# gdalsanto/flamo

Measured on AMD Instinct MI355X. Metric: freq-bin*channel products/sec (fwd+bwd), nfft=96000 8x8ch, higher is better.
Workload: dtype f32; 1 GPU; BASELINE configs[1]: Shell(FFT -> Series(Matrix 8x8, GEQ 8x8) -> iFFT), nfft=96000, batch 32 per GPU, fwd+bwd of (y**2).mean(), parameter grads; nfft=96000, channels=8, batch_per_gpu=32, parallelism=dp1 (batch), input_grad=False

## Files before the change

flamo_amd/_lib.py:

```python
from __future__ import annotations

import ctypes as C
import os
import subprocess
import threading

_HERE = os.path.dirname(os.path.abspath(__file__))
LIB_PATH = os.environ.get("FLAMO_HIP_LIB") or os.path.join(_HERE, "libflamo_hip.so")
CSRC = os.path.join(_HERE, "csrc")

_lock = threading.Lock()
_lib = None

_vp, _i, _l, _d, _sz = C.c_void_p, C.c_int, C.c_long, C.c_double, C.c_size_t

_SIGNATURES = {
    "fl_version": (_i, []),
    "fl_last_error": (C.c_char_p, []),
    "fl_twiddle_fill_f32": (_i, [_vp, _i, _vp]),
    "fl_twiddle_fill_f64": (_i, [_vp, _i, _vp]),
    "fl_fft_plan": (_i, [_i, _i, C.POINTER(_i), C.POINTER(_i)]),
    "fl_fft_scratch_elems": (_sz, [_i, _i, _i]),
    "fl_debug_set_fft_max_single": (_i, [_i]),
    "fl_debug_set_fft_fast": (_i, [_i]),
# ... 7 lines not shown
    "fl_spec_plan": (_i, [_i, C.POINTER(_i), C.POINTER(_i)]),
    "fl_spec_supports": (_i, [_i, _i, _i]),
    "fl_spec_supports_f64": (_i, [_i, _i, _i]),
    "fl_spec_aux_elems": (_sz, [_i]),
    "fl_spec_aux_fill_f32": (_i, [_vp, _i, _vp]),
    "fl_spec_aux_fill_f64": (_i, [_vp, _i, _vp]),
    "fl_debug_set_spec": (_i, [_i, _i]),
    "fl_debug_set_spec_times": (_i, [_vp]),
    "fl_spec_cols_fwd_f32": (_i, [_vp, _i, _i, _i, _vp, _vp, _i, _d, _vp]),
    "fl_spec_cols_fwd_f64": (_i, [_vp, _i, _i, _i, _vp, _vp, _i, _d, _vp]),
    "fl_spec_gradh_loop_supports_f32": (_i, [_i, _i, _i]),
    "fl_spec_gradh_loop_supports_f64": (_i, [_i, _i, _i]),
    "fl_spec_gradh_loop_f32": (_i, [_vp, _vp, _l, _l, _vp, _l, _l, _vp, _i, _i, _i, _i, _d, _i, _d, _vp, _vp]),
    "fl_spec_gradh_loop_f64": (_i, [_vp, _vp, _l, _l, _vp, _l, _l, _vp, _i, _i, _i, _i, _d, _i, _d, _vp, _vp]),
    "fl_spec_mid_f32": (_i, [_vp, _vp, _vp, _l, _l, _vp, _l, _l, _i, _vp, _i, _i, _i, _i, _d, _i, _i, _vp]),
    "fl_spec_mid_f64": (_i, [_vp, _vp, _vp, _l, _l, _vp, _l, _l, _i, _vp, _i, _i, _i, _i, _d, _i, _i, _vp]),
    "fl_spec_walk_supports": (_i, [_i, _i, _i]),
    "fl_spec_walk_spectrum_elems": (_sz, [_i, _i, _i]),
    "fl_spec_walk_workgroups": (_i, [_i, _i]),
    "fl_spec_walk_partition": (_i, [_i, _i, _i, C.POINTER(_i)]),
    "fl_spec_mid_walk_f32": (_i, [_vp, _vp, _vp, _vp, _l, _l, _i, _vp, _i, _i, _i, _i, _d, _i, _i, _vp, _vp]),
    "fl_spec_gradh_slices": (_i, [_i, _i]),
    "fl_spec_gradh_walk_f32": (_i, [_vp, _vp, _vp, _l, _l, _l, _i, _vp, _i, _i, _i, _i, _d, _i, _vp]),
    "fl_sum_parts_c64": (_i, [_vp, _l, _i, _vp, _l, _vp]),
    "fl_debug_set_walk": (_i, [_i, _i, _i, _vp]),
    "fl_debug_set_walk_stamps": (_i, [_vp]),
    "fl_wall_clock_khz": (_i, []),
    "fl_spec_cols_inv_f32": (_i, [_vp, _vp, _i, _i, _i, _i, _vp, _i, _d, _d, _vp]),
    "fl_spec_cols_inv_sumsq_f32": (_i, [_vp, _vp, _i, _i, _i, _i, _vp, _i, _d, _d, _vp, _vp]),
    "fl_spec_cols_inv_sumsq_f64": (_i, [_vp, _vp, _i, _i, _i, _i, _vp, _i, _d, _d, _vp, _vp]),
    "fl_spec_cols_blocks_f32": (_i, [_i, _i, _i]),
    "fl_spec_cols_blocks_f64": (_i, [_i, _i, _i]),
    "fl_spec_cols_inv_inplace_ok_f32": (_i, [_i, _i]),
    "fl_spec_cols_inv_inplace_ok_f64": (_i, [_i, _i]),
    "fl_spec_cols_inv_grad_supported_f32": (_i, [_i, _i]),
    "fl_spec_cols_inv_grad_supported_f64": (_i, [_i, _i]),
    "fl_spec_cols_inv_sumsq_grad_f32": (_i, [_vp, _vp, _vp, _i, _i, _vp, _i, _d, _vp, _vp]),
    "fl_spec_cols_inv_sumsq_grad_f64": (_i, [_vp, _vp, _vp, _i, _i, _vp, _i, _d, _vp, _vp]),
    "fl_spec_cols_inv_scaled_f32": (_i, [_vp, _vp, _i, _i, _i, _i, _vp, _i, _d, _vp, _d, _vp]),
    "fl_spec_cols_inv_scaled_f64": (_i, [_vp, _vp, _i, _i, _i, _i, _vp, _i, _d, _vp, _d, _vp]),
    "fl_spec_gradh_walk_scaled_f32": (_i, [_vp, _vp, _vp, _l, _l, _l, _i, _vp, _i, _i, _i, _i, _d, _i, _vp, _vp]),
    "fl_mean_square_final_f32": (_i, [_vp, _i, _d, _vp, _vp]),
    "fl_mean_square_final_f64": (_i, [_vp, _i, _d, _vp, _vp]),
    "fl_pack_toggle": (_i, [_vp, _i, _vp, _vp, _vp, _vp]),
    "fl_spec_cols_inv_f64": (_i, [_vp, _vp, _i, _i, _i, _i, _vp, _i, _d, _d, _vp]),
    "fl_permute_bins_c64": (_i, [_vp, _l, _vp, _l, _i, _i, _i, _vp]),
# ... 177 lines not shown
```

flamo_amd/csrc/specwalk.hip:

```cpp
#include "spectral_common.h"

namespace fl {
using namespace sp32;

struct WalkArgs {
    const cf* S;
    cf* S2;
    const cf* H;
    long hs_m, hs_n;
    int conj_h;
    const cf* W;
    int n, L, L1, L2, Bn;
    float spec_scale;
    int spec_interior2;
    int pre_half;
    const int* bounds;
    cf* Xp;
    long long* dbg_times;
    unsigned pol;
    long long* stamps;
};

__device__ __forceinline__ int opaque(int v) {
    asm volatile("" : "+v"(v));
// ... 392 lines not shown
        o[1] = clock64();
#pragma unroll
        for (int i = 0; i < 4; ++i) o[2 + i] = t_ph[i];
    }
    if (DBG && a.dbg_times && (tid == 0 || tid == 256))
        a.dbg_times[(size_t)blockIdx.x * 8 + 6 + grp] = grp == 0 && a.spec_interior2 == 7
            ? (q_ph[0] >> 4) | ((q_ph[1] >> 4) << 21) | ((q_ph[2] >> 4) << 42)
            : (w_ph[0] >> 4) | ((w_ph[1] >> 4) << 21) | ((w_ph[2] >> 4) << 42);
#undef FL_STAMP
}

struct GradhArgs {
    const cf* Sg;
    const cf* Xp;
    cf* dH;
    long ds_s, ds_m, ds_n;
    const cf* W;
    int n, L, L1, L2, Bn, NS;
    float scale_g;
    const float* out_scale;
    int interior2_g;
    long long* dbg_times;
    unsigned pol;
};

template <int A, int B, int NI, int NO, int NSC, int OCC, int DEPTH, bool DBG = false>
__global__ void __launch_bounds__(512, OCC) spec_gradh_walk(GradhArgs a) {
    extern __shared__ __attribute__((aligned(16))) char smem[];
    constexpr int LEN = A * B, LENP = walk_pitch(LEN);
    constexpr int NOL = NO / NSC;
    constexpr int UB = 2 * NOL * LENP;
    constexpr int NI1 = 2 * B * NOL, NI2 = 2 * NOL * A;
    constexpr int NW1 = (NI1 + 63) / 64;
    constexpr int SBG = NW1 * A * 64;
    constexpr int SBX = 8 * NI * 64;
    static_assert(LEN <= 256, "one bin pair per thread pair");
    static_assert(NO % NSC == 0 && NOL % 2 == 0 && NI % 2 == 0 && A % 2 == 0, "16-byte DMA granules");
    static_assert(NI1 <= 256 && NI2 <= 256, "an FFT stage of one unit fits one group");
    static_assert(DEPTH == 1 || DEPTH == 2, "one or two items in flight");
    constexpr int GA = A / 2, XA = NI / 2;
    constexpr int P2_OFF = 256 - ((NI2 + 63) / 64) * 64;
    cf* XF = reinterpret_cast<cf*>(smem);
    cf* Yb = XF + 2 * UB;
    cf* stage_g = Yb + UB;
    cf* stage_x = stage_g + DEPTH * SBG;
    constexpr int TWP = tw_pitch(A), TWL = (B * TWP + 1) & ~1;
    cf* tw = stage_x + DEPTH * SBX;
    cf* ws = tw + TWL;
    const int tid = threadIdx.x;
    const int wave = __builtin_amdgcn_readfirstlane(tid >> 6), lane = tid & 63;
    const int grp = wave >> 2;
    const int P = a.L1 / 2 + 1;
    const int xcd = blockIdx.x & 7, q_ = blockIdx.x >> 3;
    const int r = (q_ / (a.NS * NSC)) * 8 + xcd, sl = (q_ / NSC) % a.NS, mo = (q_ % NSC) * NOL;
    if (r >= P) return;
    const int rm = (a.L1 - r) % a.L1;
    const bool selfm = rm == r;
    const int b_lo = (int)((long)a.Bn * sl / a.NS), n_it = (int)((long)a.Bn * (sl + 1) / a.NS) - b_lo;
    const size_t bstride_g = (size_t)a.L1 * a.L2 * NO;
    const unsigned sg_lds = lds_addr_of(stage_g), sx_lds = lds_addr_of(stage_x);

    auto fetch_g = [&](int i, int cw) {
        const int b = b_lo + ((a.pol & POL_GRADH_FORWARD) ? i : n_it - 1 - i);
        const unsigned sg_buf = sg_lds + (unsigned)((i % DEPTH) * SBG * 8);
        const int hi = lane >> 5;
        int item0 = 64 * cw + 2 * (lane & 31);
        if (item0 >= NI1 || (item0 >= B * NOL && selfm)) item0 = 0;
        const int m0 = item0 % NOL, tb = (item0 / NOL) % B, slot = item0 / (NOL * B);
        const cf* src = a.Sg + (size_t)b * bstride_g + (size_t)(slot ? rm : r) * (a.L2 * NO) + ((hi * B + tb) * NO + mo + m0);
        if (a.pol & POL_GRADH_SG_NT) {
#pragma unroll
            for (int q = 0; q < A / 2; ++q) dma16p<true>(src + q * (2 * B * NO), sg_buf + (unsigned)(((cw * A + 2 * q) * 64) * 8));
        } else {
#pragma unroll
            for (int q = 0; q < A / 2; ++q) dma16p<false>(src + q * (2 * B * NO), sg_buf + (unsigned)(((cw * A + 2 * q) * 64) * 8));
        }
    };
    auto fetch_x = [&](int i, int cw) {
        const int b = b_lo + ((a.pol & POL_GRADH_FORWARD) ? i : n_it - 1 - i);
        const unsigned sx_buf = sx_lds + (unsigned)((i % DEPTH) * SBX * 8);
#if FL_XP_PAIRS
        int pp = 64 * (cw & 3) + lane;
        if (pp > LEN - 1) pp = LEN - 1;
        const cf* src = a.Xp + (((size_t)r * a.Bn + b) * 2 + (cw >> 2)) * (NI * LEN) + 2 * pp;
#else
        int pp = 64 * (cw & 3) + 2 * (lane & 31);
        if (pp > LEN - 2) pp = LEN - 2;
        const cf* src = a.Xp + (((size_t)r * a.Bn + b) * 2 + (cw >> 2)) * (NI * LEN) + (lane >> 5) * LEN + pp;
#endif
        if (a.pol & POL_GRADH_XP_NT) {
#pragma unroll
            for (int q = 0; q < NI / 2; ++q) dma16p<true>(src + q * (2 * LEN), sx_buf + (unsigned)(((cw * NI + 2 * q) * 64) * 8));
        } else {
#pragma unroll
            for (int q = 0; q < NI / 2; ++q) dma16p<false>(src + q * (2 * LEN), sx_buf + (unsigned)(((cw * NI + 2 * q) * 64) * 8));
        }
    };

    const int p = tid & 255;
    int slotB = 0, colB = 0;
    bool dc = false;
    const bool valid = p < LEN && pair_of(r, selfm, p, LEN, slotB, colB, dc);
    const int pc = p < LEN ? p : 0;
    f2 acc[NOL][NI];
#pragma unroll
    for (int m = 0; m < NOL; ++m)
#pragma unroll
        for (int nn = 0; nn < NI; ++nn) acc[m][nn] = f2{0.f, 0.f};
    const bool has_g = grp == 0 && (wave & 3) < NW1;
    const bool fetcher = DEPTH == 2 && wave >= 2 && wave <= 5;
    const int fi = wave - 2;
    const int xlo = NW1 >= 2 ? (fi == 0 ? 0 : fi == 1 ? 1 : fi == 2 ? 2 : 5) : (fi == 0 ? 0 : fi == 1 ? 1 : fi == 2 ? 3 : 6);
    const int xhi = NW1 >= 2 ? (fi == 0 ? 1 : fi == 1 ? 2 : fi == 2 ? 5 : 8) : (fi == 0 ? 1 : fi == 1 ? 3 : fi == 2 ? 6 : 8);
    int x_issued = 0;
    if (DEPTH == 2) {
        if (fetcher && fi < NW1 && n_it > 0) fetch_g(0, fi);
    } else if (has_g && n_it > 0) {
        fetch_g(0, wave & 3);
    }
    for (int j = tid; j < LEN; j += 512) {
        tw[(j / A) * TWP + j % A] = a.W[a.n + a.L1 + (j / A) * (j % A)];
        ws[j] = a.W[a.n + a.L1 + a.L2 + j];
    }
    const cf wr = a.W[r];
    lds_barrier();
    const f2 wk = v2(wr * ws[pc]);
    const f2 iws = grp ? rot_i(wk) : f2{wk.y, -wk.x}, niws = grp ? f2{-wk.x, -wk.y} : wk;
    const float hg = 0.5f * a.scale_g;
    const float sc = dc ? hg : hg * (a.interior2_g ? 2.f : 1.f);
    const f2 scv = grp ? f2{sc, -sc} : f2{sc, sc};
    const int yk_o = pc, ym_o = slotB * NOL * LENP + colB;

    long long g_ph[2] = {0, 0}, g_last = 0, g_begin = 0;
    if (DBG) g_begin = g_last = clock64();
#define FL_GSTAMP(i)                        \
    if (DBG) {                              \
        const long long t_now = clock64();  \
        g_ph[i] += t_now - g_last;          \
        g_last = t_now;                     \
    }
#pragma unroll 1
    for (int t = 0; t < n_it + 2; ++t) {
        const bool x_now = DEPTH == 1 && t >= 1 && t <= n_it;
        if (t >= 2) {
#pragma unroll
            for (int m = 0; m < NOL; ++m)
#pragma unroll
                for (int nn = 0; nn < NI; ++nn) asm volatile("" : "+v"(acc[m][nn]));
            if (DEPTH == 1) wait_vm_le((has_g && t < n_it) ? GA : 0);
        }
        f2 x[NI];
        {
#if FL_XP_PAIRS
            const f4* xs = reinterpret_cast<const f4*>(stage_x + (t % DEPTH) * SBX + (wave * NI) * 64) + lane;
#pragma unroll
            for (int j = 0; j < NI / 2; ++j) {
                const f4 q = xs[j * 64];
                x[2 * j] = f2{q.x, q.y};
// ... 63 lines not shown
#pragma unroll
                for (int tb = 0; tb < B; ++tb) v[tb] = xr[tb];
                RegFFT<float, B, false>::run(v);
                cf* yr = Yb + (slot * NOL + m) * LENP + ka;
#pragma unroll
                for (int kb = 0; kb < B; ++kb) yr[A * kb] = v[kb];
            }
        }
        long long t_work = 0;
        if (DBG) t_work = clock64() - g_last;
        lds_barrier();
        FL_GSTAMP(1)
        if (DBG && a.dbg_times && lane == 0 && (wave == 0 || wave == 1 || wave == 4 || wave == 7))
            atomicAdd((unsigned long long*)(a.dbg_times + (size_t)blockIdx.x * 8 + (wave == 0 ? 4 : wave == 1 ? 5 : wave == 4 ? 6 : 7)), (unsigned long long)t_work);
    }
#undef FL_GSTAMP
    if (DBG && a.dbg_times && tid == 0) {
        long long* o = a.dbg_times + (size_t)blockIdx.x * 8;
        o[0] = g_begin;
        o[1] = clock64();
        o[2] = g_ph[0];
        o[3] = g_ph[1];
    }
    {
        const unsigned ik = (unsigned)r * LEN + p;
        const unsigned im = dc ? (unsigned)a.L : (unsigned)(slotB ? rm : r) * LEN + colB;
        if (valid && !(grp && im == ik)) {
            cf* out = a.dH + (size_t)sl * a.ds_s;
            const unsigned bin = grp ? im : ik;
            if (a.out_scale) {
                const float os = *a.out_scale;
#pragma unroll
                for (int m = 0; m < NOL; ++m)
#pragma unroll
                    for (int nn = 0; nn < NI; ++nn) acc[m][nn] *= os;
            }
#pragma unroll
            for (int m = 0; m < NOL; ++m) {
                unsigned o = 8u * ((unsigned)(mo + m) * (unsigned)a.ds_m + bin);
                const unsigned step = 8u * (unsigned)a.ds_n;
                if (a.pol & POL_GRADH_DH_NT) {
#pragma unroll
                    for (int nn = 0; nn < NI; ++nn) {
                        st_nt(out, o, c2(acc[m][nn]));
                        o += step;
                    }
                } else {
#pragma unroll
                    for (int nn = 0; nn < NI; ++nn) {
                        at(out, o) = c2(acc[m][nn]);
                        o += step;
                    }
                }
            }
        }
    }
}

__global__ void __launch_bounds__(256) sum_parts_kernel(const float4* __restrict__ parts, long stride4, int ns, float4* __restrict__ out, long n4) {
    const long j = (long)blockIdx.x * 256 + threadIdx.x;
    if (j >= n4) return;
    float4 s = parts[j];
    for (int k = 1; k < ns; ++k) {
        const float4 v = parts[(long)k * stride4 + j];
        s.x += v.x; s.y += v.y; s.z += v.z; s.w += v.w;
    }
    out[j] = s;
}

constexpr int kMaxDevices = 64;
constexpr int kMaxWalkWgs = 1024;
static int g_walk = 1;
static int g_walk_wgs = 0;
static int g_walk_slices = 0;
static long long* g_walk_times = nullptr;
static long long* g_walk_stamps = nullptr;
static int g_walk_nsc = 2;
static int g_walk_fc = [] { const char* e = getenv("FLAMO_WALK_FC"); return e ? atoi(e) : 38; }();
static int g_walk_fc2 = [] { const char* e = getenv("FLAMO_WALK_FC2"); return e ? atoi(e) : 38; }();
static int g_walk_us = [] { const char* e = getenv("FLAMO_WALK_US"); return e ? atoi(e) : 16; }();

long long* walk_successor_stamp() { return g_walk_stamps ? g_walk_stamps + 2 * kMaxWalkWgs : nullptr; }

static int device_cus() {
    static int cus[kMaxDevices] = {};
    int dev = 0;
    if (hipGetDevice(&dev) != hipSuccess || dev < 0 || dev >= kMaxDevices) dev = 0;
    if (!cus[dev]) {
        int v = 0;
        if (hipDeviceGetAttribute(&v, hipDeviceAttributeMultiprocessorCount, dev) != hipSuccess || v <= 0) v = 256;
        cus[dev] = v;
    }
    return cus[dev];
}

static long walk_wgs(int L1, int Bn) {
    const long units = (long)(L1 / 2 + 1) * Bn;
    long g = g_walk_wgs > 0 ? g_walk_wgs : device_cus();
    if (g > units) g = units;
    if (g >= 8) g -= g % 8;
    return g;
}
// ... 37 lines not shown
    else hipLaunchKernelGGL(kern, dim3((unsigned)g), dim3(512), lds, st, a);
    return FL_OK;
}

}

using namespace fl;

extern "C" {

int fl_debug_set_walk_stamps(void* buf) {
    g_walk_stamps = (long long*)buf;
    return FL_OK;
}

int fl_wall_clock_khz(void) {
    int dev = 0, khz = 0;
    if (hipGetDevice(&dev) != hipSuccess || hipDeviceGetAttribute(&khz, hipDeviceAttributeWallClockRate, dev) != hipSuccess || khz <= 0) khz = 100000;
    return khz;
}

int fl_debug_set_walk(int mode, int wgs, int slices, void* times) {
    g_walk_nsc = mode == 14 ? 4 : mode == 15 ? 1 : 2;
    g_walk = mode;
    g_walk_wgs = wgs;
    g_walk_slices = slices;
    g_walk_times = (long long*)times;
    return FL_OK;
}

static bool walk_shape(int l2, int n_in, int n_out) {
    auto ch = [](int c) { return c == 2 || c == 4 || c == 8; };
    return (l2 == 240 || l2 == 256) && ch(n_in) && ch(n_out);
}
int fl_spec_walk_supports(int nfft, int n_in, int n_out) {
    int l1, l2;
    if (!g_walk || spec_plan(nfft, l1, l2) != FL_OK) return 0;
    if (!walk_shape(l2, n_in, n_out)) return 0;
    return walk_lds_bytes<16, 16, 8, 8>() <= device_lds_limit();
}

int fl_spec_gradh_slices(int nfft, int Bn) {
    int l1, l2;
    if (spec_plan(nfft, l1, l2) != FL_OK || Bn <= 0) return 0;
    if (g_walk_slices > 0) return g_walk_slices < Bn ? g_walk_slices : Bn;
    const int P = l1 / 2 + 1;
    int ns = device_cus() / (2 * P);
    if (g_walk_nsc == 4) ns = 1;
    if (g_walk_nsc == 1) ns = device_cus() / P;
    if (ns < 1) ns = 1;
    return ns < Bn ? ns : Bn;
}

static int gradh_walk_impl(const void* Sg, const void* Xp, void* dH_parts, long ds_s, long ds_m, long ds_n, int n_slices, const void* W,
                           int nfft, int Bn, int NI, int NO, double scale_g, int interior2_g, const float* out_scale, void* stream);
int fl_spec_gradh_walk_f32(const void* Sg, const void* Xp, void* dH_parts, long ds_s, long ds_m, long ds_n, int n_slices, const void* W,
                           int nfft, int Bn, int NI, int NO, double scale_g, int interior2_g, void* stream) {
    return gradh_walk_impl(Sg, Xp, dH_parts, ds_s, ds_m, ds_n, n_slices, W, nfft, Bn, NI, NO, scale_g, interior2_g, nullptr, stream);
}
int fl_spec_gradh_walk_scaled_f32(const void* Sg, const void* Xp, void* dH_parts, long ds_s, long ds_m, long ds_n, int n_slices, const void* W,
                                  int nfft, int Bn, int NI, int NO, double scale_g, int interior2_g, const void* out_scale, void* stream) {
    return gradh_walk_impl(Sg, Xp, dH_parts, ds_s, ds_m, ds_n, n_slices, W, nfft, Bn, NI, NO, scale_g, interior2_g, (const float*)out_scale, stream);
}
}
static int gradh_walk_impl(const void* Sg, const void* Xp, void* dH_parts, long ds_s, long ds_m, long ds_n, int n_slices, const void* W,
                           int nfft, int Bn, int NI, int NO, double scale_g, int interior2_g, const float* out_scale, void* stream) {
    FL_REQUIRE(Sg && Xp && dH_parts && W, "spec_gradh_walk: null pointer");
    FL_REQUIRE(n_slices >= 1 && n_slices <= (Bn > 0 ? Bn : 1), "spec_gradh_walk: slices must be in [1, batch]");
    FL_REQUIRE(reinterpret_cast<uintptr_t>(Sg) % 16 == 0 && reinterpret_cast<uintptr_t>(Xp) % 16 == 0, "spec_gradh_walk: scratch arrays must be 16-byte aligned");
    if (Bn == 0) return FL_OK;
    GradhArgs a = {};
    int rc = spec_plan(nfft, a.L1, a.L2);
    if (rc) return rc;
    a.Sg = (const cf*)Sg; a.Xp = (const cf*)Xp; a.dH = (cf*)dH_parts; a.ds_s = ds_s; a.ds_m = ds_m; a.ds_n = ds_n;
    a.W = (const cf*)W; a.n = nfft; a.L = nfft / 2; a.Bn = Bn; a.NS = n_slices;
    a.scale_g = (float)scale_g; a.interior2_g = interior2_g; a.dbg_times = g_walk_times; a.out_scale = out_scale;
    a.pol = stream_policy();
    FL_REQUIRE((size_t)NO * (size_t)ds_m * 8ull < (1ull << 32), "spec_gradh_walk: a partial plane set exceeds 32-bit offsets");
    const int P = a.L1 / 2 + 1;
    hipStream_t st = (hipStream_t)stream;
    int lrc = FL_ERR_UNSUPPORTED;
#define FL_GRADH(A_, B_, NI_, NO_, NSC_, OCC_, DEPTH_)                                                                            \
    {                                                                                                                            \
        constexpr int LEN = A_ * B_, LENP = walk_pitch(LEN), NOL = NO_ / NSC_;                                                   \
        constexpr size_t lds = ((size_t)3 * 2 * NOL * LENP + DEPTH_ * (((2 * B_ * NOL + 63) / 64) * A_ * 64 + 8 * NI_ * 64) +    \
                                ((B_ * tw_pitch(A_) + 1) & ~1) + LEN) * sizeof(cf);                                              \
        static_assert(lds <= 160 * 1024, "LDS budget");                                                                          \
        const unsigned nblk = (unsigned)(cdiv_i(P, 8) * 8 * n_slices * NSC_);                                                    \
        auto kern = spec_gradh_walk<A_, B_, NI_, NO_, NSC_, OCC_, DEPTH_>;                                                       \
        auto kern_dbg = spec_gradh_walk<A_, B_, NI_, NO_, NSC_, OCC_, DEPTH_, true>;                                             \
        static bool done[kMaxDevices] = {}, done_dbg[kMaxDevices] = {};                                                          \
        lrc = ensure_lds(reinterpret_cast<const void*>(kern), lds, done);                                                        \
        if (!lrc && a.dbg_times) lrc = ensure_lds(reinterpret_cast<const void*>(kern_dbg), lds, done_dbg);                       \
        if (!lrc) {                                                                                                              \
            if (a.dbg_times) hipLaunchKernelGGL(kern_dbg, dim3(nblk), dim3(512), lds, st, a);                                    \
            else hipLaunchKernelGGL(kern, dim3(nblk), dim3(512), lds, st, a);                                                    \
        }                                                                                                                        \
    }
#define FL_GRADH_ROWS(A_, B_)                                                                                                    \
    if (NI == 8 && NO == 8) {                                                                                                    \
        if (A_ == 16 && B_ == 15 && g_walk_nsc == 4) FL_GRADH(16, 15, 8, 8, 4, 4, 1)                                             \
        else if (A_ == 16 && B_ == 15 && g_walk_nsc == 1) FL_GRADH(16, 15, 8, 8, 1, 2, 1)                                        \
        else if (A_ == 16 && B_ == 15 && g_walk == 17) FL_GRADH(16, 15, 8, 8, 2, 2, 1)                                           \
        else FL_GRADH(A_, B_, 8, 8, 2, 2, 2)                                                                                     \
    }                                                                                                                            \
    else if (NI == 4 && NO == 8) FL_GRADH(A_, B_, 4, 8, 2, 2, 1)                                                                 \
    else if (NI == 2 && NO == 8) FL_GRADH(A_, B_, 2, 8, 2, 2, 1)                                                                 \
    else if (NI == 8 && NO == 4) FL_GRADH(A_, B_, 8, 4, 2, 2, 1)                                                                 \
    else if (NI == 4 && NO == 4) FL_GRADH(A_, B_, 4, 4, 2, 2, 1)                                                                 \
    else if (NI == 2 && NO == 4) FL_GRADH(A_, B_, 2, 4, 2, 2, 1)                                                                 \
    else if (NI == 8 && NO == 2) FL_GRADH(A_, B_, 8, 2, 1, 2, 1)                                                                 \
    else if (NI == 4 && NO == 2) FL_GRADH(A_, B_, 4, 2, 1, 2, 1)                                                                 \
    else if (NI == 2 && NO == 2) FL_GRADH(A_, B_, 2, 2, 1, 2, 1)
    if (a.L2 == 240) { FL_GRADH_ROWS(16, 15) }
    else if (a.L2 == 256) { FL_GRADH_ROWS(16, 16) }
#undef FL_GRADH_ROWS
// ... 115 lines not shown
```

flamo_amd/ops.py:

```python
from __future__ import annotations

import math
import threading
from collections import namedtuple
from typing import NamedTuple, Optional, Tuple

import torch

from . import _lib

__all__ = ["rfft", "irfft", "spectral_apply", "permute_bins", "mimo", "solve", "delay_response", "sos_response", "geq_sections", "solve_dud", "to_planar", "set_bin_shard",
           "bin_shard"]


def _require_gpu(*ts: torch.Tensor) -> torch.device:
    dev = None
    for t in ts:
        if t is None:
            continue
        if not t.is_cuda:
            raise RuntimeError(
                "flamo_amd: tensors must live on a ROCm device (got %s); the HIP path has no CPU fallback" % t.device
            )
        dev = t.device if dev is None else dev
# ... 832 lines not shown
                   "spec_mid_walk")
    return S2, Xp


INVERSE_IN_PLACE = True
GRADH_LOOP = True
GRADH_LOOP_MAX_BATCH = 4


def _spec_gradh_loop(Sg, Xs, B, NI, NO, nfft, scale_g, host_factor, out_scale):
    dev = Sg.device
    M = nfft // 2 + 1
    real = _rdtype(Sg)
    P = _pitch(M)
    dH = _empty_rows((NO, NI), M, Sg.dtype, dev)
    with kernel_timer.span("spec_gradh_loop"):
        _lib.check(_spec_fn("fl_spec_gradh_loop", real)(Sg.data_ptr(), Xs.data_ptr(), NI * P, P, dH.data_ptr(), NI * P, P,
                                                        twiddles(nfft, real, dev).data_ptr(), nfft, B, NI, NO, float(scale_g), 1,
                                                        float(host_factor), None if out_scale is None else out_scale.data_ptr(),
                                                        _stream()), "spec_gradh_loop")
    return dH.movedim(-1, 0)


def _spec_gradh_walk(Sg, Xp, B, NI, NO, nfft, scale_g, out_scale=None):
    dev = Sg.device
    L = _lib.lib()
    M = nfft // 2 + 1
    P = _pitch(M)
    ns = int(L.fl_spec_gradh_slices(nfft, B))
    parts = torch.empty((ns, NO, NI, P), dtype=torch.complex64, device=dev)
    with kernel_timer.span("spec_gradh_walk"):
        _lib.check(L.fl_spec_gradh_walk_scaled_f32(Sg.data_ptr(), Xp.data_ptr(), parts.data_ptr(), NO * NI * P, NI * P, P, ns,
                                                   twiddles(nfft, torch.float32, dev).data_ptr(), nfft, B, NI, NO, scale_g, 1,
                                                   None if out_scale is None else out_scale.data_ptr(), _stream()),
                   "spec_gradh_walk")
    if ns == 1:
        out = parts[0]
    else:
        out = torch.empty((NO, NI, P), dtype=torch.complex64, device=dev)
        with kernel_timer.span("sum_parts"):
            _lib.check(L.fl_sum_parts_c64(parts.data_ptr(), NO * NI * P, ns, out.data_ptr(), NO * NI * P, _stream()), "sum_parts")
    return out[..., :M].movedim(-1, 0)


class _SpectralApply(torch.autograd.Function):
    @staticmethod
    def forward(ctx, x, Hrm, nfft, scale_f, env_f, scale_i, env_i):
        _require_gpu(x, Hrm)
        if x.dtype not in (torch.float32, torch.float64) or x.dim() != 3:
            raise TypeError("spectral_apply expects a real float32 / float64 (B, T, N) signal")
        M = nfft // 2 + 1
# ... 1658 lines not shown
```

include/flamo_hip.h:

```cpp
#ifndef FLAMO_HIP_H
#define FLAMO_HIP_H

#include <stddef.h>
#include <stdint.h>

#ifdef __cplusplus
extern "C" {
#endif

#define FL_OK 0
#define FL_ERR_BAD_ARG (-1)
#define FL_ERR_UNSUPPORTED (-2)
#define FL_ERR_HIP (-3)

#define FL_ABI_VERSION 1

int fl_version(void);
const char* fl_last_error(void);


int fl_twiddle_fill_f32(void* W, int nfft, void* stream);
int fl_twiddle_fill_f64(void* W, int nfft, void* stream);

int fl_fft_plan(int nfft, int is_f64, int* L1, int* L2);
// ... 21 lines not shown
int fl_spec_plan(int nfft, int* L1, int* L2);
size_t fl_spec_aux_elems(int nfft);
int fl_spec_aux_fill_f32(void* W, int nfft, void* stream);
int fl_spec_supports(int nfft, int n_in, int n_out);
int fl_debug_set_spec(int vt, int rg);
int fl_debug_set_spec_times(void* buf);
int fl_spec_cols_fwd_f32(const void* x, int Bn, int t_len, int G, void* S, const void* W, int nfft, double env_log2,
                         void* stream);
int fl_spec_mid_f32(const void* S, void* S2, void* Xs, long xs_b, long xs_n, const void* H, long hs_m, long hs_n, int conj_h,
                    const void* W, int nfft, int Bn, int NI, int NO, double spec_scale, int spec_interior2, int pre_half,
                    void* stream);
int fl_spec_walk_supports(int nfft, int n_in, int n_out);
size_t fl_spec_walk_spectrum_elems(int nfft, int Bn, int NI);
int fl_spec_walk_workgroups(int nfft, int Bn);
int fl_spec_walk_partition(int nfft, int Bn, int n_wg, int* bounds);
int fl_spec_mid_walk_f32(const void* S, void* S2, void* Xp, const void* H, long hs_m, long hs_n, int conj_h, const void* W, int nfft, int Bn,
                         int NI, int NO, double spec_scale, int spec_interior2, int pre_half, const void* bounds, void* stream);
int fl_spec_gradh_slices(int nfft, int Bn);
int fl_spec_gradh_walk_f32(const void* Sg, const void* Xp, void* dH_parts, long ds_s, long ds_m, long ds_n, int n_slices, const void* W,
                           int nfft, int Bn, int NI, int NO, double scale_g, int interior2_g, void* stream);
int fl_spec_gradh_walk_scaled_f32(const void* Sg, const void* Xp, void* dH_parts, long ds_s, long ds_m, long ds_n, int n_slices,
                                  const void* W, int nfft, int Bn, int NI, int NO, double scale_g, int interior2_g,
                                  const void* out_scale, void* stream);
int fl_sum_parts_c64(const void* parts, long part_stride, int n_parts, void* out, long n, void* stream);
int fl_debug_set_walk(int mode, int wgs, int slices, void* times);
int fl_debug_set_walk_stamps(void* buf);
int fl_wall_clock_khz(void);
int fl_spec_cols_inv_f32(const void* S2, void* y, int Bn, int t_len, int t_out, int G, const void* W, int nfft, double scale,
                         double env_log2, void* stream);
int fl_spec_cols_inv_sumsq_f32(const void* S2, void* y, int Bn, int t_len, int t_out, int G, const void* W, int nfft, double scale,
                               double env_log2, void* sumsq_parts, void* stream);
int fl_spec_cols_blocks_f32(int nfft, int Bn, int G);
int fl_spec_cols_inv_grad_supported_f32(int nfft, int G);
int fl_spec_cols_inv_inplace_ok_f32(int nfft, int G);
int fl_spec_cols_inv_sumsq_grad_f32(const void* S2, void* y, void* Sg, int Bn, int G, const void* W, int nfft, double scale,
                                    void* sumsq_parts, void* stream);
int fl_spec_cols_inv_scaled_f32(const void* S2, void* y, int Bn, int t_len, int t_out, int G, const void* W, int nfft, double scale,
                                const void* dev_scale, double env_log2, void* stream);
int fl_permute_bins_c64(const void* src, long src_pitch, void* dst, long dst_pitch, int nplanes, int nfft, int inverse,
                        void* stream);
int fl_spec_gradh_loop_supports_f32(int nfft, int NI, int NO);
int fl_spec_gradh_loop_supports_f64(int nfft, int NI, int NO);
int fl_spec_gradh_loop_f32(const void* Sg, const void* Xs, long xs_b, long xs_n, void* dH, long ds_m, long ds_n, const void* W,
                           int nfft, int Bn, int NI, int NO, double scale_g, int interior2, double out_scale,
                           const void* dev_scale, void* stream);
int fl_spec_gradh_loop_f64(const void* Sg, const void* Xs, long xs_b, long xs_n, void* dH, long ds_m, long ds_n, const void* W,
// ... 303 lines not shown
```

Baseline: 675.0 billion products/s.

## Balance gradient-H walk with a per-CU work partition and in-kernel slab reduction

Replaces the fixed grid of (row, batch-slice, output-half) blocks in the gradient-of-H walk kernel with a host-built partition. The partition spreads row×batch work units evenly across one workgroup per CU. When a task is split across several workgroups, each writes its partial accumulator to a slab and uses an atomic ticket, so the last arriver sums the slabs and stores the final plane. This removes the separate partial-sum buffer and the sum_parts pass, and targets load imbalance. In exchange it adds a ticket memset, slab traffic, cross-workgroup ordering on atomics, and cached plan tables built on first use.

```diff
diff --git a/flamo_amd/_lib.py b/flamo_amd/_lib.py
--- a/flamo_amd/_lib.py
+++ b/flamo_amd/_lib.py
@@ -53,6 +53,9 @@
     "fl_spec_mid_walk_f32": (_i, [_vp, _vp, _vp, _vp, _l, _l, _i, _vp, _i, _i, _i, _i, _d, _i, _i, _vp, _vp]),
     "fl_spec_gradh_slices": (_i, [_i, _i]),
     "fl_spec_gradh_walk_f32": (_i, [_vp, _vp, _vp, _l, _l, _l, _i, _vp, _i, _i, _i, _i, _d, _i, _vp]),
+    "fl_spec_gradh_partition": (_i, [_i, _i, _i, _i, _i, C.POINTER(_i), C.POINTER(_i), C.POINTER(_i)]),
+    "fl_spec_gradh_walk_ws_bytes": (_sz, [_i, _i, _i, _i]),
+    "fl_spec_gradh_walk_part_f32": (_i, [_vp, _vp, _vp, _l, _l, _vp, _i, _i, _i, _i, _d, _i, _vp, _vp, _vp, _vp, _sz, _vp]),
     "fl_sum_parts_c64": (_i, [_vp, _l, _i, _vp, _l, _vp]),
     "fl_debug_set_walk": (_i, [_i, _i, _i, _vp]),
     "fl_debug_set_walk_stamps": (_i, [_vp]),
diff --git a/flamo_amd/csrc/specwalk.hip b/flamo_amd/csrc/specwalk.hip
--- a/flamo_amd/csrc/specwalk.hip
+++ b/flamo_amd/csrc/specwalk.hip
@@ -1,4 +1,11 @@
 #include "spectral_common.h"
+
+#include <algorithm>
+#include <array>
+#include <map>
+#include <memory>
+#include <mutex>
+#include <vector>
 
 namespace fl {
 using namespace sp32;
@@ -438,9 +445,27 @@
     int interior2_g;
     long long* dbg_times;
     unsigned pol;
+    const int* bounds;
+    const int* tasks;
+    unsigned* tickets;
+    float* slabs;
+    int lanes, wg_sub;
 };
 
-template <int A, int B, int NI, int NO, int NSC, int OCC, int DEPTH, bool DBG = false>
+typedef unsigned u4 __attribute__((ext_vector_type(4)));
+constexpr int kAuxSc1 = 16;
+__device__ __forceinline__ __amdgpu_buffer_rsrc_t slab_rsrc(float* base, unsigned bytes) {
+    return __builtin_amdgcn_make_buffer_rsrc(base, 0, (int)bytes, 0x00020000);
+}
+__device__ __forceinline__ void slab_store(__amdgpu_buffer_rsrc_t rs, unsigned byte_off, f2 lo, f2 hi) {
+    const u4 q = {__float_as_uint(lo.x), __float_as_uint(lo.y), __float_as_uint(hi.x), __float_as_uint(hi.y)};
+    __builtin_amdgcn_raw_buffer_store_b128(q, rs, (int)byte_off, 0, kAuxSc1);
+}
+__device__ __forceinline__ u4 slab_load(__amdgpu_buffer_rsrc_t rs, unsigned byte_off) {
+    return __builtin_amdgcn_raw_buffer_load_b128(rs, (int)byte_off, 0, kAuxSc1);
+}
+
+template <int A, int B, int NI, int NO, int NSC, int OCC, int DEPTH, bool PART, bool DBG = false>
 __global__ void __launch_bounds__(512, OCC) spec_gradh_walk(GradhArgs a) {
     extern __shared__ __attribute__((aligned(16))) char smem[];
     constexpr int LEN = A * B, LENP = walk_pitch(LEN);
@@ -468,16 +493,43 @@
     const int grp = wave >> 2;
     const int P = a.L1 / 2 + 1;
     const int xcd = blockIdx.x & 7, q_ = blockIdx.x >> 3;
-    const int r = (q_ / (a.NS * NSC)) * 8 + xcd, sl = (q_ / NSC) % a.NS, mo = (q_ % NSC) * NOL;
-    if (r >= P) return;
+    int v_wg = 0, u_seg = 0, u_hi = 0;
+    if constexpr (PART) {
+        const int lane_x = a.lanes == 8 ? xcd : 0, ql = a.lanes == 8 ? q_ : (int)blockIdx.x;
+        v_wg = (lane_x * NSC + ql % NSC) * a.wg_sub + ql / NSC;
+        u_seg = a.bounds[v_wg];
+        u_hi = a.bounds[v_wg + 1];
+        if (u_seg >= u_hi) return;
+    }
+    const size_t bstride_g = (size_t)a.L1 * a.L2 * NO;
+    const unsigned sg_lds = lds_addr_of(stage_g), sx_lds = lds_addr_of(stage_x);
+    long long g_ph[2] = {0, 0}, g_last = 0, g_begin = 0;
+    if (DBG) g_begin = g_last = clock64();
+    bool first_seg = true;
+    do {
+    int r, sl = 0, mo, b_lo = 0, n_it, i0 = 0;
+    int4 tk = {0, 0, 0, 0};
+    if constexpr (PART) {
+        const int T = u_seg / a.Bn, u_end = min(u_hi, (T + 1) * a.Bn);
+        tk = reinterpret_cast<const int4*>(a.tasks)[T];
+        r = tk.x & 0xFFFFFF;
+        mo = (tk.x >> 24) * NOL;
+        i0 = u_seg - T * a.Bn;
+        n_it = u_end - u_seg;
+    } else {
+        r = (q_ / (a.NS * NSC)) * 8 + xcd, sl = (q_ / NSC) % a.NS, mo = (q_ % NSC) * NOL;
+        if (r >= P) return;
+        b_lo = (int)((long)a.Bn * sl / a.NS), n_it = (int)((long)a.Bn * (sl + 1) / a.NS) - b_lo;
+    }
     const int rm = (a.L1 - r) % a.L1;
     const bool selfm = rm == r;
-    const int b_lo = (int)((long)a.Bn * sl / a.NS), n_it = (int)((long)a.Bn * (sl + 1) / a.NS) - b_lo;
-    const size_t bstride_g = (size_t)a.L1 * a.L2 * NO;
-    const unsigned sg_lds = lds_addr_of(stage_g), sx_lds = lds_addr_of(stage_x);
+    auto item_b = [&](int i) {
+        if constexpr (PART) return (a.pol & POL_GRADH_FORWARD) ? i0 + i : a.Bn - 1 - (i0 + i);
+        else return b_lo + ((a.pol & POL_GRADH_FORWARD) ? i : n_it - 1 - i);
+    };
 
     auto fetch_g = [&](int i, int cw) {
-        const int b = b_lo + ((a.pol & POL_GRADH_FORWARD) ? i : n_it - 1 - i);
+        const int b = item_b(i);
         const unsigned sg_buf = sg_lds + (unsigned)((i % DEPTH) * SBG * 8);
         const int hi = lane >> 5;
         int item0 = 64 * cw + 2 * (lane & 31);
@@ -493,7 +545,7 @@
         }
     };
     auto fetch_x = [&](int i, int cw) {
-        const int b = b_lo + ((a.pol & POL_GRADH_FORWARD) ? i : n_it - 1 - i);
+        const int b = item_b(i);
         const unsigned sx_buf = sx_lds + (unsigned)((i % DEPTH) * SBX * 8);
 #if FL_XP_PAIRS
         int pp = 64 * (cw & 3) + lane;
@@ -534,9 +586,11 @@
     } else if (has_g && n_it > 0) {
         fetch_g(0, wave & 3);
     }
-    for (int j = tid; j < LEN; j += 512) {
-        tw[(j / A) * TWP + j % A] = a.W[a.n + a.L1 + (j / A) * (j % A)];
-        ws[j] = a.W[a.n + a.L1 + a.L2 + j];
+    if (!PART || first_seg) {
+        for (int j = tid; j < LEN; j += 512) {
+            tw[(j / A) * TWP + j % A] = a.W[a.n + a.L1 + (j / A) * (j % A)];
+            ws[j] = a.W[a.n + a.L1 + a.L2 + j];
+        }
     }
     const cf wr = a.W[r];
     lds_barrier();
@@ -547,9 +601,7 @@
     const f2 scv = grp ? f2{sc, -sc} : f2{sc, sc};
     const int yk_o = pc, ym_o = slotB * NOL * LENP + colB;
 
-    long long g_ph[2] = {0, 0}, g_last = 0, g_begin = 0;
-    if (DBG) g_begin = g_last = clock64();
-#define FL_GSTAMP(i)                        \
+#define FL_GSTAMP(i)                      \
     if (DBG) {                              \
         const long long t_now = clock64();  \
         g_ph[i] += t_now - g_last;          \
@@ -659,7 +711,7 @@
         o[2] = g_ph[0];
         o[3] = g_ph[1];
     }
-    {
+    auto store_plane = [&](f2 (&v)[NOL][NI]) {
         const unsigned ik = (unsigned)r * LEN + p;
         const unsigned im = dc ? (unsigned)a.L : (unsigned)(slotB ? rm : r) * LEN + colB;
         if (valid && !(grp && im == ik)) {
@@ -670,7 +722,7 @@
 #pragma unroll
                 for (int m = 0; m < NOL; ++m)
 #pragma unroll
-                    for (int nn = 0; nn < NI; ++nn) acc[m][nn] *= os;
+                    for (int nn = 0; nn < NI; ++nn) v[m][nn] *= os;
             }
 #pragma unroll
             for (int m = 0; m < NOL; ++m) {
@@ -679,19 +731,80 @@
                 if (a.pol & POL_GRADH_DH_NT) {
 #pragma unroll
                     for (int nn = 0; nn < NI; ++nn) {
-                        st_nt(out, o, c2(acc[m][nn]));
+                        st_nt(out, o, c2(v[m][nn]));
                         o += step;
                     }
                 } else {
 #pragma unroll
                     for (int nn = 0; nn < NI; ++nn) {
-                        at(out, o) = c2(acc[m][nn]);
+                        at(out, o) = c2(v[m][nn]);
                         o += step;
                     }
                 }
             }
         }
-    }
+    };
+    const int n_parts = PART ? (int)((unsigned)tk.y >> 24) : 1;
+    if (!PART || n_parts == 1) {
+        store_plane(acc);
+    } else {
+        constexpr unsigned SLAB = (unsigned)(NOL * NI) * 8u * 512u, RUN = 16u * 512u;
+        const int part = v_wg - (tk.y & 0xFFFFFF);
+        const __amdgpu_buffer_rsrc_t rs = slab_rsrc(a.slabs + (size_t)tk.w * (SLAB / 4), (unsigned)n_parts * SLAB);
+        const unsigned lane_off = 16u * (unsigned)tid;
+#pragma unroll
+        for (int m = 0; m < NOL; ++m)
+#pragma unroll
+            for (int nn = 0; nn < NI; nn += 2)
+                slab_store(rs, (unsigned)part * SLAB + (unsigned)((m * NI + nn) / 2) * RUN + lane_off, acc[m][nn], acc[m][nn + 1]);
+        asm volatile("s_waitcnt vmcnt(0)" ::: "memory");
+        lds_barrier();
+        int* const told = reinterpret_cast<int*>(Yb);
+        if (tid == 0) *told = (int)__hip_atomic_fetch_add(a.tickets + tk.z, 1u, __ATOMIC_RELAXED, __HIP_MEMORY_SCOPE_AGENT);
+        lds_barrier();
+        const bool last = __builtin_amdgcn_readfirstlane(*told) == n_parts - 1;
+        if (last) {
+            __builtin_amdgcn_fence(__ATOMIC_ACQUIRE, "wavefront");
+            f2 sum[NOL][NI];
+#pragma unroll
+            for (int m = 0; m < NOL; ++m)
+#pragma unroll
+                for (int nn = 0; nn < NI; ++nn) sum[m][nn] = f2{0.f, 0.f};
+#pragma unroll 1
+            for (int pp = 0; pp < n_parts; ++pp) {
+                f2 t[NOL][NI];
+                if (pp == part) {
+#pragma unroll
+                    for (int m = 0; m < NOL; ++m)
+#pragma unroll
+                        for (int nn = 0; nn < NI; ++nn) t[m][nn] = acc[m][nn];
+                } else {
+                    u4 q[NOL * NI / 2];
+#pragma unroll
+                    for (int j = 0; j < NOL * NI / 2; ++j) q[j] = slab_load(rs, (unsigned)pp * SLAB + (unsigned)j * RUN + lane_off);
+#pragma unroll
+                    for (int m = 0; m < NOL; ++m)
+#pragma unroll
+                        for (int nn = 0; nn < NI; nn += 2) {
+                            const u4 w = q[(m * NI + nn) / 2];
+                            t[m][nn] = f2{__uint_as_float(w.x), __uint_as_float(w.y)};
+                            t[m][nn + 1] = f2{__uint_as_float(w.z), __uint_as_float(w.w)};
+                        }
+                }
+#pragma unroll
+                for (int m = 0; m < NOL; ++m)
+#pragma unroll
+                    for (int nn = 0; nn < NI; ++nn) sum[m][nn] = pp == 0 ? t[m][nn] : sum[m][nn] + t[m][nn];
+            }
+            store_plane(sum);
+        }
+    }
+    if constexpr (PART) {
+        u_seg += n_it;
+        first_seg = false;
+    }
+    } while (PART && u_seg < u_hi);
+    if (PART && DBG && a.dbg_times && tid == 0) a.dbg_times[(size_t)blockIdx.x * 8 + 1] = clock64();
 }
 
 __global__ void __launch_bounds__(256) sum_parts_kernel(const float4* __restrict__ parts, long stride4, int ns, float4* __restrict__ out, long n4) {
@@ -715,6 +828,11 @@
 static int g_walk_nsc = 2;
 static int g_walk_fc = [] { const char* e = getenv("FLAMO_WALK_FC"); return e ? atoi(e) : 38; }();
 static int g_walk_fc2 = [] { const char* e = getenv("FLAMO_WALK_FC2"); return e ? atoi(e) : 38; }();
+#ifndef FL_GRADH_PARTITION_DEFAULT
+#define FL_GRADH_PARTITION_DEFAULT 1
+#endif
+static int g_gradh_part_env = [] { const char* e = getenv("FLAMO_GRADH_PARTITION"); return e ? atoi(e) : FL_GRADH_PARTITION_DEFAULT; }();
+static int g_gradh_part = g_gradh_part_env;
 static int g_walk_us = [] { const char* e = getenv("FLAMO_WALK_US"); return e ? atoi(e) : 16; }();
 
 long long* walk_successor_stamp() { return g_walk_stamps ? g_walk_stamps + 2 * kMaxWalkWgs : nullptr; }
@@ -798,6 +916,7 @@
 
 int fl_debug_set_walk(int mode, int wgs, int slices, void* times) {
     g_walk_nsc = mode == 14 ? 4 : mode == 15 ? 1 : 2;
+    g_gradh_part = mode == 18 ? 0 : mode == 19 ? 1 : g_gradh_part_env;
     g_walk = mode;
     g_walk_wgs = wgs;
     g_walk_slices = slices;
@@ -828,8 +947,132 @@
     return ns < Bn ? ns : Bn;
 }
 
+struct GradhPlan {
+    int nsc = 0, lanes = 0, wg_sub = 0, n_wg = 0, n_tasks = 0, n_cut = 0, n_slabs = 0, max_parts = 0, max_range = 0;
+    std::vector<int> bounds, tasks;
+};
+
+static int gradh_plan_build(int nfft, int Bn, int NI, int NO, int n_wg, GradhPlan& pl) {
+    int L1, L2;
+    if (spec_plan(nfft, L1, L2) != FL_OK || !walk_shape(L2, NI, NO) || Bn < 4) return FL_ERR_UNSUPPORTED;
+    const int P = L1 / 2 + 1, NSC = NO == 2 ? 1 : 2;
+    const long units = (long)P * NSC * Bn;
+    if (n_wg <= 0) n_wg = device_cus();
+    if (n_wg > units) n_wg = (int)units;
+    if (n_wg >= 8) n_wg -= n_wg % 8;
+    const int LX = n_wg >= 8 * NSC ? 8 : 1, M = n_wg / (LX * NSC);
+    if (M < 1) return FL_ERR_UNSUPPORTED;
+    pl.nsc = NSC; pl.lanes = LX; pl.wg_sub = M; pl.n_wg = n_wg; pl.n_tasks = P * NSC;
+    pl.bounds.assign(n_wg + 1, (int)units);
+    pl.tasks.assign(4 * (size_t)pl.n_tasks, 0);
+    int t_first = 0;
+    for (int s = 0; s < LX * NSC; ++s) {
+        const int x = s / NSC, g = s % NSC, K = x < P ? (P - x + LX - 1) / LX : 0, U = K * Bn;
+        std::vector<int> b(M + 1, U);
+        if (K > 0 && M <= K) {
+            for (int j = 0; j < M; ++j) b[j] = (int)((long)j * U / M);
+        } else if (K > 0) {
+            int c = M / K, e = M - c * K;
+            if (c >= FL_GRADH_MAX_PARTS) c = FL_GRADH_MAX_PARTS, e = 0;
+            const int groups = e > 0 ? e : K;
+            int pos = 0, t0 = 0;
+            for (int i = 0; i < groups; ++i) {
+                const int k = e > 0 ? K / e + (i < K % e ? 1 : 0) : 1, w = e > 0 ? c * k + 1 : c;
+                for (int j = 0; j < w; ++j) b[pos + j] = t0 * Bn + (int)((long)j * k * Bn / w);
+                pos += w;
+                t0 += k;
+            }
+        }
+        const int v0 = s * M, u0 = t_first * Bn;
+        bool ended = false;
+        for (int j = 0; j < M; ++j) {
+            pl.bounds[v0 + j] = u0 + b[j];
+            const int len = b[j + 1] - b[j];
+            if (len < 0 || (len > 0 && ended)) return FL_ERR_UNSUPPORTED;
+            ended = ended || len == 0;
+            if (len > pl.max_range) pl.max_range = len;
+        }
+        pl.bounds[v0 + M] = u0 + U;
+        for (int k = 0, j = 0; k < K; ++k) {
+            while (b[j + 1] <= k * Bn) ++j;
+            int parts = 1;
+            while (b[j + parts] < (k + 1) * Bn) ++parts;
+            if (parts > FL_GRADH_MAX_PARTS) return FL_ERR_UNSUPPORTED;
+            int* t = &pl.tasks[4 * (size_t)(t_first + k)];
+            t[0] = (LX * k + x) | (g << 24);
+            t[1] = (v0 + j) | (parts << 24);
+            t[2] = parts > 1 ? pl.n_cut : -1;
+            t[3] = parts > 1 ? pl.n_slabs : 0;
+            if (parts > 1) ++pl.n_cut, pl.n_slabs += parts;
+            if (parts > pl.max_parts) pl.max_parts = parts;
+        }
+        t_first += K;
+    }
+    return FL_OK;
+}
+static const GradhPlan* gradh_plan(int nfft, int Bn, int NI, int NO, int n_wg) {
+    static std::mutex mu;
+    static std::map<std::array<int, 5>, std::unique_ptr<GradhPlan>> plans;
+    if (n_wg <= 0) n_wg = device_cus();
+    std::lock_guard<std::mutex> lock(mu);
+    auto& slot = plans[{nfft, Bn, NI, NO, n_wg}];
+    if (!slot) {
+        slot.reset(new GradhPlan);
+        if (gradh_plan_build(nfft, Bn, NI, NO, n_wg, *slot) != FL_OK) slot->n_wg = 0;
+    }
+    return slot->n_wg > 0 ? slot.get() : nullptr;
+}
+static size_t gradh_ticket_bytes(const GradhPlan& pl) { return ((size_t)pl.n_cut * 4 + 255) / 256 * 256; }
+static size_t gradh_slab_bytes(int NI, int NO, int nsc) { return (size_t)(NO / nsc) * NI * 8 * 512; }
+static bool gradh_part_on() { return g_gradh_part != 0 && g_walk_nsc == 2 && g_walk != 17 && g_walk_slices == 0; }
+
+int fl_spec_gradh_partition(int nfft, int Bn, int NI, int NO, int n_wg, int* bounds, int* tasks, int* info) {
+    FL_REQUIRE(n_wg >= 0, "spec_gradh_partition: bad arguments");
+    const GradhPlan* pl = gradh_plan(nfft, Bn, NI, NO, n_wg);
+    if (!pl) {
+        set_error("spec_gradh_partition: nfft=%d, batch %d, %d -> %d channels on %d workgroups has no partition", nfft, Bn, NI, NO, n_wg);
+        return FL_ERR_UNSUPPORTED;
+    }
+    if (bounds) {
+        const int n = n_wg > 0 ? n_wg : pl->n_wg;
+        for (int i = 0; i <= n; ++i) bounds[i] = pl->bounds[i < pl->n_wg ? i : pl->n_wg];
+    }
+    if (tasks) std::copy(pl->tasks.begin(), pl->tasks.end(), tasks);
+    if (info) {
+        const int v[8] = {pl->n_wg, pl->n_tasks, pl->n_cut, pl->n_slabs, pl->max_parts, pl->max_range, pl->lanes, pl->wg_sub};
+        std::copy(v, v + 8, info);
+    }
+    return FL_OK;
+}
+
+size_t fl_spec_gradh_walk_ws_bytes(int nfft, int Bn, int NI, int NO) {
+    if (!gradh_part_on()) return 0;
+    const GradhPlan* pl = gradh_plan(nfft, Bn, NI, NO, 0);
+    if (!pl) return 0;
+    return gradh_ticket_bytes(*pl) + (size_t)pl->n_slabs * gradh_slab_bytes(NI, NO, pl->nsc) + 256;
+}
+
+struct GradhPart {
+    const GradhPlan* pl;
+    const int *bounds, *tasks;
+    void* ws;
+};
 static int gradh_walk_impl(const void* Sg, const void* Xp, void* dH_parts, long ds_s, long ds_m, long ds_n, int n_slices, const void* W,
-                           int nfft, int Bn, int NI, int NO, double scale_g, int interior2_g, const float* out_scale, void* stream);
+                           int nfft, int Bn, int NI, int NO, double scale_g, int interior2_g, const float* out_scale, void* stream,
+                           const GradhPart* part = nullptr);
+int fl_spec_gradh_walk_part_f32(const void* Sg, const void* Xp, void* dH, long ds_m, long ds_n, const void* W, int nfft, int Bn, int NI, int NO,
+                                double scale_g, int interior2_g, const void* out_scale, const void* bounds, const void* tasks, void* ws,
+                                size_t ws_bytes, void* stream) {
+    FL_REQUIRE(bounds && tasks && ws && reinterpret_cast<uintptr_t>(ws) % 256 == 0, "spec_gradh_walk_part: tables and a 256-byte aligned workspace are required");
+    const GradhPlan* pl = gradh_plan(nfft, Bn, NI, NO, 0);
+    if (!pl) {
+        set_error("spec_gradh_walk_part: nfft=%d, batch %d, %d -> %d channels has no partition", nfft, Bn, NI, NO);
+        return FL_ERR_UNSUPPORTED;
+    }
+    FL_REQUIRE(ws_bytes >= gradh_ticket_bytes(*pl) + (size_t)pl->n_slabs * gradh_slab_bytes(NI, NO, pl->nsc), "spec_gradh_walk_part: workspace too small");
+    const GradhPart part = {pl, (const int*)bounds, (const int*)tasks, ws};
+    return gradh_walk_impl(Sg, Xp, dH, 0, ds_m, ds_n, 1, W, nfft, Bn, NI, NO, scale_g, interior2_g, (const float*)out_scale, stream, &part);
+}
 int fl_spec_gradh_walk_f32(const void* Sg, const void* Xp, void* dH_parts, long ds_s, long ds_m, long ds_n, int n_slices, const void* W,
                            int nfft, int Bn, int NI, int NO, double scale_g, int interior2_g, void* stream) {
     return gradh_walk_impl(Sg, Xp, dH_parts, ds_s, ds_m, ds_n, n_slices, W, nfft, Bn, NI, NO, scale_g, interior2_g, nullptr, stream);
@@ -840,7 +1083,8 @@
 }
 }
 static int gradh_walk_impl(const void* Sg, const void* Xp, void* dH_parts, long ds_s, long ds_m, long ds_n, int n_slices, const void* W,
-                           int nfft, int Bn, int NI, int NO, double scale_g, int interior2_g, const float* out_scale, void* stream) {
+                           int nfft, int Bn, int NI, int NO, double scale_g, int interior2_g, const float* out_scale, void* stream,
+                           const GradhPart* part) {
     FL_REQUIRE(Sg && Xp && dH_parts && W, "spec_gradh_walk: null pointer");
     FL_REQUIRE(n_slices >= 1 && n_slices <= (Bn > 0 ? Bn : 1), "spec_gradh_walk: slices must be in [1, batch]");
     FL_REQUIRE(reinterpret_cast<uintptr_t>(Sg) % 16 == 0 && reinterpret_cast<uintptr_t>(Xp) % 16 == 0, "spec_gradh_walk: scratch arrays must be 16-byte aligned");
@@ -856,18 +1100,30 @@
     const int P = a.L1 / 2 + 1;
     hipStream_t st = (hipStream_t)stream;
     int lrc = FL_ERR_UNSUPPORTED;
+    if (part) {
+        const size_t tb = gradh_ticket_bytes(*part->pl);
+        a.bounds = part->bounds; a.tasks = part->tasks; a.lanes = part->pl->lanes; a.wg_sub = part->pl->wg_sub;
+        a.tickets = (unsigned*)part->ws;
+        a.slabs = (float*)((char*)part->ws + tb);
+        if (tb && hipMemsetAsync(part->ws, 0, tb, st) != hipSuccess) {
+            set_error("spec_gradh_walk: clearing the ticket words failed");
+            return FL_ERR_HIP;
+        }
+    }
 #define FL_GRADH(A_, B_, NI_, NO_, NSC_, OCC_, DEPTH_)                                                                            \
     {                                                                                                                            \
         constexpr int LEN = A_ * B_, LENP = walk_pitch(LEN), NOL = NO_ / NSC_;                                                   \
         constexpr size_t lds = ((size_t)3 * 2 * NOL * LENP + DEPTH_ * (((2 * B_ * NOL + 63) / 64) * A_ * 64 + 8 * NI_ * 64) +    \
                                 ((B_ * tw_pitch(A_) + 1) & ~1) + LEN) * sizeof(cf);                                              \
         static_assert(lds <= 160 * 1024, "LDS budget");                                                                          \
-        const unsigned nblk = (unsigned)(cdiv_i(P, 8) * 8 * n_slices * NSC_);                                                    \
-        auto kern = spec_gradh_walk<A_, B_, NI_, NO_, NSC_, OCC_, DEPTH_>;                                                       \
-        auto kern_dbg = spec_gradh_walk<A_, B_, NI_, NO_, NSC_, OCC_, DEPTH_, true>;                                             \
-        static bool done[kMaxDevices] = {}, done_dbg[kMaxDevices] = {};                                                          \
-        lrc = ensure_lds(reinterpret_cast<const void*>(kern), lds, done);                                                        \
-        if (!lrc && a.dbg_times) lrc = ensure_lds(reinterpret_cast<const void*>(kern_dbg), lds, done_dbg);                       \
+        const unsigned nblk = part ? (unsigned)(a.lanes * NSC_ * a.wg_sub) : (unsigned)(cdiv_i(P, 8) * 8 * n_slices * NSC_);     \
+        constexpr bool PK = NSC_ == (NO_ == 2 ? 1 : 2);       \
+        auto kern = part ? spec_gradh_walk<A_, B_, NI_, NO_, NSC_, OCC_, DEPTH_, PK> : spec_gradh_walk<A_, B_, NI_, NO_, NSC_, OCC_, DEPTH_, false>; \
+        auto kern_dbg = part ? spec_gradh_walk<A_, B_, NI_, NO_, NSC_, OCC_, DEPTH_, PK, true>                                   \
+                             : spec_gradh_walk<A_, B_, NI_, NO_, NSC_, OCC_, DEPTH_, false, true>;                               \
+        static bool done[2][kMaxDevices] = {}, done_dbg[2][kMaxDevices] = {};                                                    \
+        lrc = part && part->pl->nsc != NSC_ ? FL_ERR_UNSUPPORTED : ensure_lds(reinterpret_cast<const void*>(kern), lds, done[part ? 1 : 0]); \
+        if (!lrc && a.dbg_times) lrc = ensure_lds(reinterpret_cast<const void*>(kern_dbg), lds, done_dbg[part ? 1 : 0]);         \
         if (!lrc) {                                                                                                              \
             if (a.dbg_times) hipLaunchKernelGGL(kern_dbg, dim3(nblk), dim3(512), lds, st, a);                                    \
             else hipLaunchKernelGGL(kern, dim3(nblk), dim3(512), lds, st, a);                                                    \
diff --git a/flamo_amd/ops.py b/flamo_amd/ops.py
--- a/flamo_amd/ops.py
+++ b/flamo_amd/ops.py
@@ -878,11 +878,45 @@
     return dH.movedim(-1, 0)
 
 
+_gradh_tables = {}
+_gradh_last_ws = None
+
+
+def _gradh_partition(nfft: int, B: int, NI: int, NO: int, dev: torch.device):
+    key = (int(nfft), int(B), int(NI), int(NO), dev.index if dev.index is not None else torch.cuda.current_device())
+    t = _gradh_tables.get(key)
+    if t is None:
+        if torch.cuda.is_current_stream_capturing():
+            return None
+        import ctypes
+        L = _lib.lib()
+        info = (ctypes.c_int * 8)()
+        _lib.check(L.fl_spec_gradh_partition(nfft, B, NI, NO, 0, None, None, info), "spec_gradh_partition")
+        bounds, tasks = (ctypes.c_int * (info[0] + 1))(), (ctypes.c_int * (4 * info[1]))()
+        _lib.check(L.fl_spec_gradh_partition(nfft, B, NI, NO, 0, bounds, tasks, None), "spec_gradh_partition")
+        t = (torch.tensor(list(bounds), dtype=torch.int32).to(dev), torch.tensor(list(tasks), dtype=torch.int32).to(dev))
+        torch.cuda.current_stream(dev).synchronize()
+        _gradh_tables[key] = t
+    return t
+
+
 def _spec_gradh_walk(Sg, Xp, B, NI, NO, nfft, scale_g, out_scale=None):
     dev = Sg.device
     L = _lib.lib()
     M = nfft // 2 + 1
     P = _pitch(M)
+    ws_bytes = int(L.fl_spec_gradh_walk_ws_bytes(nfft, B, NI, NO))
+    tables = _gradh_partition(nfft, B, NI, NO, dev) if ws_bytes else None
+    if tables is not None:
+        global _gradh_last_ws
+        out = torch.empty((NO, NI, P), dtype=torch.complex64, device=dev)
+        ws = _gradh_last_ws = torch.empty(ws_bytes, dtype=torch.uint8, device=dev)
+        with kernel_timer.span("spec_gradh_walk"):
+            _lib.check(L.fl_spec_gradh_walk_part_f32(Sg.data_ptr(), Xp.data_ptr(), out.data_ptr(), NI * P, P,
+                                                     twiddles(nfft, torch.float32, dev).data_ptr(), nfft, B, NI, NO, scale_g, 1,
+                                                     None if out_scale is None else out_scale.data_ptr(), tables[0].data_ptr(),
+                                                     tables[1].data_ptr(), ws.data_ptr(), ws_bytes, _stream()), "spec_gradh_walk_part")
+        return out[..., :M].movedim(-1, 0)
     ns = int(L.fl_spec_gradh_slices(nfft, B))
     parts = torch.empty((ns, NO, NI, P), dtype=torch.complex64, device=dev)
     with kernel_timer.span("spec_gradh_walk"):
diff --git a/include/flamo_hip.h b/include/flamo_hip.h
--- a/include/flamo_hip.h
+++ b/include/flamo_hip.h
@@ -67,6 +67,12 @@
 int fl_spec_gradh_walk_scaled_f32(const void* Sg, const void* Xp, void* dH_parts, long ds_s, long ds_m, long ds_n, int n_slices,
                                   const void* W, int nfft, int Bn, int NI, int NO, double scale_g, int interior2_g,
                                   const void* out_scale, void* stream);
+#define FL_GRADH_MAX_PARTS 4
+int fl_spec_gradh_partition(int nfft, int Bn, int NI, int NO, int n_wg, int* bounds, int* tasks, int* info);
+size_t fl_spec_gradh_walk_ws_bytes(int nfft, int Bn, int NI, int NO);
+int fl_spec_gradh_walk_part_f32(const void* Sg, const void* Xp, void* dH, long ds_m, long ds_n, const void* W, int nfft, int Bn, int NI,
+                                int NO, double scale_g, int interior2_g, const void* out_scale, const void* bounds, const void* tasks,
+                                void* ws, size_t ws_bytes, void* stream);
 int fl_sum_parts_c64(const void* parts, long part_stride, int n_parts, void* out, long n, void* stream);
 int fl_debug_set_walk(int mode, int wgs, int slices, void* times);
 int fl_debug_set_walk_stamps(void* buf);
```

After: 629.4 billion products/s. -6.8%, worse.
